# intuitive-robots/mdt_policy

Measured on AMD Instinct MI355X. Metric: action-chunks/sec (10-step denoise, horizon=10), higher is better.
Workload: dtype f32

## Files before the change

include/mdt_hip_ops.h:

```cpp
#ifndef MDT_HIP_OPS_H
#define MDT_HIP_OPS_H

#include <stdint.h>
#include "mdt_hip.h"

#ifdef __cplusplus
extern "C" {
#endif

enum { MDT_ACT_NONE = 0, MDT_ACT_GELU = 1, MDT_ACT_MISH = 2, MDT_ACT_SILU = 3,
       MDT_ACT_SWIGLU = 4  };
enum { MDT_HEAD_DENOISED = 0, MDT_HEAD_DDIM = 1, MDT_HEAD_RAW = 2,
       MDT_HEAD_PLAN = 3  };

int64_t mdt_op_packed_numel(int64_t N, int64_t K);

mdt_status mdt_op_pack_weight(const float *w, int64_t n_rows, int64_t K, float *packed, int64_t n_off,
                              int64_t N_total, void *stream);
mdt_status mdt_op_pack_weight_glu(const float *w, int64_t H2, int64_t K, float *packed, void *stream);

typedef struct {
    const float *A;
    int64_t lda;
    const float *Wp;
    const float *bias;
    float *out;
    int64_t ldo;
    int32_t M, N, K;
    int32_t ln;
    const float *ln_w, *ln_b;
    const float *mod;
    int64_t mod_stride;
    int32_t shift_off, scale_off;
    int32_t rows_per_sample;
    int32_t act;
    int32_t residual;
    int32_t gate_off;
    int32_t gin, gout, goff;
    const float *rowvec;
    int32_t batch;
    int64_t bs_a, bs_w, bs_out;
    const float *aux;
    int32_t aux_mode;
    int32_t a_parts;
    int64_t a_part_stride;
    float *a_merged;
    const void *Wp_split;
} mdt_gemm_args;

mdt_status mdt_op_gemm(const mdt_gemm_args *args, void *stream);

mdt_status mdt_op_mlp(const mdt_gemm_args *fc, const mdt_gemm_args *proj, float *parts, int64_t part_stride,
                      int32_t *n_parts, void *stream);
mdt_status mdt_op_pack_weight_split(const float *w, int64_t n_rows, int64_t K, void *image, void *stream);
mdt_status mdt_op_pack_weight_split_rows(const float *w, int64_t n_rows, int64_t K, void *image, int64_t n_off, void *stream);
mdt_status mdt_op_mlp_split(const mdt_gemm_args *fc, const mdt_gemm_args *proj, const void *fc_split, const void *proj_split,
                            float *parts, int64_t part_stride, int32_t *n_parts, void *stream);
void mdt_op_set_mlp_split(int32_t on);
void mdt_op_set_mlp_fuse_min(int32_t rows);
void mdt_op_set_side_jobs(int32_t on);
int64_t mdt_op_side_jobs_paired(void);
void mdt_op_trace_mlp(int32_t enable);
int32_t mdt_op_trace_mlp_read(float *us, int32_t cap);
int32_t mdt_op_trace_mlp_read_empty(float *us, int32_t cap);
mdt_status mdt_op_clock_stamp(uint64_t *out16, void *stream);
void mdt_op_set_ws_split(int32_t on);

void mdt_op_set_mlp_skew(int32_t v);

void mdt_op_set_gemm_geometry(int32_t geometry);

typedef struct {
    const float *q; int64_t ldq;
    const float *k; const float *v;
    int64_t ldkv;
    float *out; int64_t ldo;
    int32_t B, H, hd, Tq, Tk;
    int32_t causal;
    int32_t rope;
} mdt_attn_args;

mdt_status mdt_op_attention(const mdt_attn_args *args, void *stream);

mdt_status mdt_op_attn_proj(const mdt_gemm_args *proj, const float *qkv, int64_t ldq, int32_t hd, int32_t T, int32_t causal,
                            void *stream);
void mdt_op_set_attn_wide_min(int32_t rows);

mdt_status mdt_op_layernorm(const float *in, const float *w, const float *b, float *out, int64_t M, int32_t D,
                            void *stream);

typedef struct {
    const float *y;
    const float *ln_w;
    const float *ln_b;
    const float *Wp, *bp;
    const float *x;
    const float *sigma;
    int64_t sigma_stride;
    float *out;
    int32_t M, D, A, rows_per_sample;
    int32_t mode;
    const float *step;
    float sigma_data;
    float *y_next;
    const float *Wa, *ba;
    int32_t no_ln;
    int32_t y_parts;
    int64_t y_part_stride;
} mdt_head_args;

mdt_status mdt_op_head(const mdt_head_args *args, void *stream);

typedef struct {
    const float *kv; int64_t ldkv;
    const float *WqT_p;
    const float *bq;
    const float *Wo_p;
    float *U, *Wf;
    float *c;
    int32_t B, H, hd, D, Te;
} mdt_xfold_args;
mdt_status mdt_op_xattn_fold(const mdt_xfold_args *args, void *stream);

typedef struct {
    float *y;
    const float *ln_w, *ln_b;
    const float *U, *Wf, *c;
    const float *bo;
    int32_t B, H, D, Te, Ta;
    float *y_out;
} mdt_xapply_args;
mdt_status mdt_op_xattn_apply(const mdt_xapply_args *args, void *stream);

mdt_status mdt_op_xattn_gemm(const mdt_xapply_args *x, const mdt_gemm_args *g, void *stream);

mdt_status mdt_op_attn_xattn(const mdt_gemm_args *proj, const float *qkv, int64_t ldq, const mdt_xapply_args *x, int32_t hd,
                             int32_t T, void *stream);

mdt_status mdt_op_action_embed(const float *x, const float *sigma, int64_t sigma_stride, float sigma_data,
                               const float *WaT, const float *ba, float *y, int64_t M, int32_t A, int32_t D,
                               int32_t rows_per_sample, void *stream);
// ... 6 lines not shown
```

mdt_policy_amd/_lib.py:

```python
from __future__ import annotations

import ctypes as C
import os
import threading

from . import build as _build

c_float_p = C.POINTER(C.c_float)


class MDTHipError(RuntimeError):
    def __init__(self, status: int, message: str):
        super().__init__(f"libmdt_hip status {status}: {message}")
        self.status = status


class MDTConfig(C.Structure):
    _fields_ = [(n, C.c_int32) for n in (
        "arch", "embed_dim", "n_heads", "n_enc_layers", "n_dec_layers", "action_dim", "obs_dim", "goal_dim",
        "n_obs_token", "goal_seq_len", "action_seq_len", "use_mlp_goal", "use_modality_encoder", "use_abs_pos_emb",
        "use_rot_embed", "use_ada_conditioning", "use_noise_encoder", "linear_output", "bias")] + [
        ("sigma_data", C.c_float), ("no_goal_conditioning", C.c_int32), ("proprio_dim", C.c_int32),
        ("use_proprio", C.c_int32)]

# ... 146 lines not shown
class MapPoolConfig(C.Structure):
    _fields_ = [(n, C.c_int32) for n in ("n_latents", "embed_dim", "output_dim", "n_heads", "mlp_hidden")]


class InfoNCEArgs(C.Structure):
    _fields_ = [("image_features", C.c_void_p), ("lang_features", C.c_void_p), ("logit_scale", C.c_void_p),
                ("batch", C.c_int32), ("dim", C.c_int32), ("mode", C.c_int32), ("loss", C.c_void_p),
                ("d_image", C.c_void_p), ("d_lang", C.c_void_p), ("d_logit_scale", C.c_void_p), ("scratch", C.c_void_p)]


INFONCE_MODE = {"symmetric": 0, "img_to_text": 1, "text_to_img": 2}
ARCH = {"mdtv": 0, "mdt": 1}
MODALITY = {"vis": 0, "lang": 1}
ACT = {"none": 0, "gelu": 1, "mish": 2, "silu": 3, "swiglu": 4}
HEAD = {"denoised": 0, "ddim": 1, "raw": 2}
RAW_OUTPUT, RAW_INPUT, SIGMA_SCALAR = 1, 2, 4

_VP, _I32, _I64, _F = C.c_void_p, C.c_int32, C.c_int64, C.c_float
SYMBOLS = [
    ("mdt_last_error", C.c_char_p, []),
    ("mdt_version", C.c_char_p, []),
    ("mdt_set_allocator", _I32, [_VP, _VP, _VP]),
    ("mdt_allocator_detach", _I32, []),
    ("mdt_create", _I32, [C.POINTER(MDTConfig), C.POINTER(_VP)]),
    ("mdt_destroy", _I32, [_VP]),
    ("mdt_param_count", _I64, [_VP]),
    ("mdt_param_name", C.c_char_p, [_VP, _I64]),
    ("mdt_param_numel", _I64, [_VP, _I64]),
    ("mdt_load_param", _I32, [_VP, C.c_char_p, _VP, _I64, _VP]),
    ("mdt_load_params", _I32, [_VP, _I32, C.POINTER(C.c_char_p), C.POINTER(C.c_void_p), C.POINTER(_I64), _VP]),
    ("mdt_reserve", _I32, [_VP, _I64]),
    ("mdt_ws_generation", _I64, [_VP]),
    ("mdt_encode", _I32, [_VP, _VP, _VP, _VP, _I32, _I32, _VP, _I64, _VP, _VP]),
    ("mdt_denoise_cached", _I32, [_VP, _VP, _VP, _I64, _I32, _VP, _VP]),
    ("mdt_forward", _I32, [_VP, _VP, _VP, _VP, _I32, _VP, _VP, _I64, _VP, _VP, _VP]),
    ("mdt_sample_ddim", _I32, [_VP, _VP, _VP, _VP, _I32, _VP, C.POINTER(C.c_float), _I32, _I64, _VP, _VP, _VP]),
    ("mdt_sample_ddim_dev", _I32, [_VP, _VP, _VP, _VP, _I32, _VP, _VP, _I32, _I64, _VP, _VP, _VP]),
    ("mdt_sample", _I32, [_VP, _VP, _VP, _VP, _I32, _VP, _I32, C.POINTER(SamplerParams), C.POINTER(C.c_float), _I32, _VP, _I32,
                          _I64, _VP, _VP, _VP]),
    ("mdt_sample_dev", _I32, [_VP, _VP, _VP, _VP, _I32, _VP, _I32, C.POINTER(SamplerParams), _VP, _I32, _VP, _I32, _I64, _VP,
                              _VP, _VP]),
    ("mdt_sampler_plan", _I32, [_I32, C.POINTER(SamplerParams), C.POINTER(C.c_float), _I32, C.POINTER(SamplerPlan)]),
    ("mdt_sample_dpm_adaptive", _I32, [_VP, _VP, _VP, _VP, _I32, _VP, C.c_float, C.c_float, C.POINTER(DpmAdaptiveParams), _I64,
                                       _VP, _VP, C.POINTER(DpmAdaptiveInfo), _VP]),
    ("mdt_sample_ddim_guided", _I32, [_VP, _VP, _VP, _VP, _I32, _VP, C.POINTER(C.c_float), _I32, _I64, _VP, _VP, _F, _VP]),
    ("mdt_sample_ddim_dev_guided", _I32, [_VP, _VP, _VP, _VP, _I32, _VP, _VP, _I32, _I64, _VP, _VP, _F, _VP]),
    ("mdt_sample_guided", _I32, [_VP, _VP, _VP, _VP, _I32, _VP, _I32, C.POINTER(SamplerParams), C.POINTER(C.c_float), _I32, _VP,
                                 _I32, _I64, _VP, _VP, _F, _VP]),
    ("mdt_sample_dev_guided", _I32, [_VP, _VP, _VP, _VP, _I32, _VP, _I32, C.POINTER(SamplerParams), _VP, _I32, _VP, _I32, _I64,
                                     _VP, _VP, _F, _VP]),
    ("mdt_brownian_noise", _I32, [_VP, _I32, C.c_double, C.c_double, C.c_double, _VP, _I32, _I64, _I64, _VP, _VP]),
    ("mdt_brownian_noise_host", _I32, [_VP, _I32, C.c_double, C.c_double, C.c_double, _VP, _I32, _I64, _I64, _VP]),
    ("mdt_sample_sde_tree", _I32, [_VP, _VP, _VP, _VP, _I32, _VP, C.POINTER(SamplerParams), C.POINTER(C.c_float), _I32,
                                   C.POINTER(BrownianSource), _I64, _VP, _VP, _VP]),
    ("mdt_sample_sde_tree_dev", _I32, [_VP, _VP, _VP, _VP, _I32, _VP, C.POINTER(SamplerParams), _VP, _I32, C.POINTER(BrownianSource),
                                       _I64, _VP, _VP, _VP]),
    ("mdt_sample_sde_tree_guided", _I32, [_VP, _VP, _VP, _VP, _I32, _VP, C.POINTER(SamplerParams), C.POINTER(C.c_float), _I32,
                                          C.POINTER(BrownianSource), _I64, _VP, _VP, _F, _VP]),
    ("mdt_sample_sde_tree_dev_guided", _I32, [_VP, _VP, _VP, _VP, _I32, _VP, C.POINTER(SamplerParams), _VP, _I32,
                                              C.POINTER(BrownianSource), _I64, _VP, _VP, _F, _VP]),
    ("mdt_sample_dpm_adaptive_guided", _I32, [_VP, _VP, _VP, _VP, _I32, _VP, C.c_float, C.c_float, C.POINTER(DpmAdaptiveParams),
                                              _I64, _VP, _VP, _F, C.POINTER(DpmAdaptiveInfo), _VP]),
    ("mdt_dpm_control_init", _I32, [C.POINTER(DpmControl)] + [C.c_double] * 6),
    ("mdt_dpm_control_update", _I32, [C.POINTER(DpmControl), C.c_float, C.POINTER(C.c_int32)]),
    ("mdt_dpm_adaptive_plan", _I32, [_I32, C.c_float, C.c_float, C.POINTER(SamplerPlan)]),
    ("mdt_op_trace_mlp", None, [_I32]),
    ("mdt_op_trace_mlp_read", _I32, [_VP, _I32]),
    ("mdt_op_trace_mlp_read_empty", _I32, [_VP, _I32]),
    ("mdt_op_clock_stamp", _I32, [_VP, _VP]),
    ("mdt_op_set_ws_split", None, [_I32]),
    ("mdt_op_set_tn_split", None, [_I32]),
    ("mdt_loss_fwd", _I32, [_VP, _VP, _VP, _VP, _I32, _VP, _VP, _VP, _I64, _VP, _VP, _VP, _VP]),
    ("mdt_flops_per_chunk", C.c_double, [_VP, _I32]),
    ("mdt_fnv1_32", C.c_uint32, [C.c_char_p, C.c_uint64, C.c_uint32]),
    ("mdt_op_packed_numel", _I64, [_I64, _I64]),
    ("mdt_op_pack_weight", _I32, [_VP, _I64, _I64, _VP, _I64, _I64, _VP]),
    ("mdt_op_pack_weight_glu", _I32, [_VP, _I64, _I64, _VP, _VP]),
    ("mdt_op_gemm", _I32, [C.POINTER(GemmArgs), _VP]),
    ("mdt_op_mlp", _I32, [C.POINTER(GemmArgs), C.POINTER(GemmArgs), _VP, _I64, C.POINTER(_I32), _VP]),
    ("mdt_op_pack_weight_split", _I32, [_VP, _I64, _I64, _VP, _VP]),
    ("mdt_op_pack_weight_split_rows", _I32, [_VP, _I64, _I64, _VP, _I64, _VP]),
    ("mdt_op_mlp_split", _I32, [C.POINTER(GemmArgs), C.POINTER(GemmArgs), _VP, _VP, _VP, _I64, C.POINTER(_I32), _VP]),
    ("mdt_op_set_mlp_split", None, [_I32]),
    ("mdt_op_set_gemm_geometry", None, [_I32]),
    ("mdt_op_set_mlp_fuse_min", None, [_I32]),
    ("mdt_op_set_side_jobs", None, [_I32]),
    ("mdt_op_side_jobs_paired", _I64, []),
    ("mdt_op_set_mlp_skew", None, [_I32]),
    ("mdt_op_set_attn_wide_min", None, [_I32]),
    ("mdt_op_attention", _I32, [C.POINTER(AttnArgs), _VP]),
    ("mdt_op_attn_proj", _I32, [C.POINTER(GemmArgs), _VP, _I64, _I32, _I32, _I32, _VP]),
    ("mdt_op_xattn_fold", _I32, [C.POINTER(XFoldArgs), _VP]),
    ("mdt_op_xattn_apply", _I32, [C.POINTER(XApplyArgs), _VP]),
    ("mdt_op_attn_xattn", _I32, [C.POINTER(GemmArgs), _VP, _I64, C.POINTER(XApplyArgs), _I32, _I32, _VP]),
    ("mdt_op_xattn_gemm", _I32, [C.POINTER(XApplyArgs), C.POINTER(GemmArgs), _VP]),
    ("mdt_op_layernorm", _I32, [_VP, _VP, _VP, _VP, _I64, _I32, _VP]),
    ("mdt_op_head", _I32, [C.POINTER(HeadArgs), _VP]),
    ("mdt_op_action_embed", _I32, [_VP, _VP, _I64, _F, _VP, _VP, _VP, _I64, _I32, _I32, _I32, _VP]),
    ("mdt_train_prepare", _I32, [_VP]),
    ("mdt_grad_numel", _I64, [_VP]),
    ("mdt_grad_offset", _I64, [_VP, _I64]),
    ("mdt_train_loss_fwd", _I32, [_VP, _VP, _VP, _VP, _I32, _VP, _VP, _VP, _I64, C.POINTER(Dropout), _VP, _VP, _VP,
                                  C.POINTER(_I32), _VP]),
    ("mdt_train_loss_bwd", _I32, [_VP, _I32, _VP, _VP, _VP, _VP, _VP, _VP, _VP]),
    ("mdt_train_loss_bwd_stages", _I32, [_VP]),
    ("mdt_train_loss_bwd_stage", _I32, [_VP, _I32, _I32, _VP, _VP, _VP, _VP, _VP, _VP, _VP]),
    ("mdt_train_param_stage", _I32, [_VP, _I64]),
    ("mdt_train_encode_fwd", _I32, [_VP, _VP, _VP, _VP, _I32, _I32, _VP, _I64, C.POINTER(Dropout), _VP, C.POINTER(_I32),
                                    _VP]),
    ("mdt_train_encode_bwd", _I32, [_VP, _I32, _VP, _VP, _VP, _VP, _VP, _VP]),
    ("mdt_tape_release", _I32, [_VP, _I32]),
    ("mdt_denoise_vjp", _I32, [_VP, _VP, _VP, _VP, _I32, _VP, _VP, _VP, _I64, _VP, _VP, _VP]),
    ("mdt_train_denoise_fwd", _I32, [_VP, _VP, _VP, _VP, _I64, C.POINTER(Dropout), _VP, C.POINTER(_I32), _VP]),
    ("mdt_train_denoise_bwd", _I32, [_VP, _I32, _VP, _VP, _VP, _VP, _VP, _VP]),
    ("mdt_op_pack_weight_t", _I32, [_VP, _I64, _I64, _I64, _VP, _I64, _I64, _VP]),
    ("mdt_op_pack_many", _I32, [_I32, C.POINTER(C.c_void_p), C.POINTER(_I32), C.POINTER(_I32), C.POINTER(C.c_void_p),
                                C.POINTER(C.c_void_p), _VP]),
    ("mdt_op_ln_fwd_train", _I32, [C.POINTER(LnTrainArgs), _VP]),
    ("mdt_op_ln_bwd", _I32, [C.POINTER(LnBwdArgs), _VP]),
    ("mdt_op_attn_bwd", _I32, [C.POINTER(AttnBwdArgs), _VP]),
    ("mdt_op_act_fwd", _I32, [_VP, _VP, _I64, _I32, _VP]),
    ("mdt_op_act_bwd", _I32, [_VP, _VP, _VP, _I64, _I32, _VP]),
    ("mdt_op_attn_fwd_train", _I32, [C.POINTER(AttnTrainArgs), _VP]),
    ("mdt_op_merge_fwd", _I32, [C.POINTER(MergeArgs), _VP]),
    ("mdt_op_merge_bwd", _I32, [C.POINTER(MergeArgs), _VP]),
    ("mdt_op_merge_ln_fwd", _I32, [C.POINTER(MergeArgs), C.POINTER(LnTrainArgs), _VP]),
    ("mdt_op_ln_bwd_merge", _I32, [C.POINTER(LnBwdArgs), C.POINTER(MergeArgs), _VP]),
    ("mdt_op_colsum", _I32, [_VP, _I64, _I64, _I64, _VP, _I32, _VP]),
    ("mdt_op_linear_bwd", _I32, [C.POINTER(LinearBwdArgs), _VP]),
    ("mdt_op_linear_bwd_scratch", _I64, [_I64, _I64, _I64]),
    ("mdt_op_linear_bwd_scratch_exact", _I64, [_I64, _I64, _I64]),
    ("mdt_op_multi_adamw", _I32, [C.POINTER(OptTensor), _I32, _F, _F, _F, _F, _F, _I64, _VP]),
    ("mdt_op_multi_ema", _I32, [C.POINTER(OptTensor), _I32, _F, _VP]),
    ("mdt_op_multi_sumsq_scratch", _I64, [C.POINTER(OptTensor), _I32]),
    ("mdt_op_multi_sumsq", _I32, [C.POINTER(OptTensor), _I32, _I32, _VP, _VP, _I64, _VP]),
    ("mdt_op_multi_adamw_dev", _I32, [C.POINTER(OptTensor), _I32, _F, _F, _F, _F, _F, _VP, _VP, _VP, _VP, _F, _VP, _VP]),
    ("mdt_resampler_create", _I32, [C.POINTER(ResamplerConfig), C.POINTER(_VP)]),
    ("mdt_resampler_destroy", _I32, [_VP]),
    ("mdt_resampler_param_count", _I64, [_VP]),
    ("mdt_resampler_param_name", C.c_char_p, [_VP, _I64]),
    ("mdt_resampler_param_numel", _I64, [_VP, _I64]),
    ("mdt_resampler_load_param", _I32, [_VP, C.c_char_p, _VP, _I64, _VP]),
    ("mdt_resampler_forward", _I32, [_VP, _VP, _VP, _I64, _I32, _I32, _VP, _VP]),
    ("mdt_resampler_train_prepare", _I32, [_VP]),
    ("mdt_resampler_grad_numel", _I64, [_VP]),
    ("mdt_resampler_grad_offset", _I64, [_VP, _I64]),
    ("mdt_resampler_forward_train", _I32, [_VP, _VP, _VP, _I64, _I32, _I32, _VP, C.POINTER(_I32), _VP]),
    ("mdt_resampler_backward", _I32, [_VP, _I32, _VP, _VP, _VP, _VP]),
    ("mdt_resampler_tape_release", _I32, [_VP, _I32]),
    ("mdt_resampler_flops", C.c_double, [_VP, _I32, _I32]),
    ("mdt_map_pool_create", _I32, [C.POINTER(MapPoolConfig), C.POINTER(_VP)]),
    ("mdt_map_pool_destroy", _I32, [_VP]),
    ("mdt_map_pool_param_count", _I64, [_VP]),
    ("mdt_map_pool_param_name", C.c_char_p, [_VP, _I64]),
    ("mdt_map_pool_param_numel", _I64, [_VP, _I64]),
    ("mdt_map_pool_load_param", _I32, [_VP, C.c_char_p, _VP, _I64, _VP]),
    ("mdt_map_pool_forward", _I32, [_VP, _VP, _I64, _I32, _VP, _VP]),
    ("mdt_map_pool_train_prepare", _I32, [_VP]),
    ("mdt_map_pool_grad_numel", _I64, [_VP]),
    ("mdt_map_pool_grad_offset", _I64, [_VP, _I64]),
    ("mdt_map_pool_forward_train", _I32, [_VP, _VP, _I64, _I32, _VP, C.POINTER(_I32), _VP]),
    ("mdt_map_pool_backward", _I32, [_VP, _I32, _VP, _VP, _VP, _VP]),
    ("mdt_map_pool_tape_release", _I32, [_VP, _I32]),
    ("mdt_op_rms_fwd", _I32, [_VP, _VP, _VP, _I64, _I32, _F, _VP]),
    ("mdt_op_rms_bwd_scratch", _I64, [_I64, _I32]),
    ("mdt_op_rms_bwd", _I32, [_VP, _VP, _VP, _VP, _I32, _VP, _I32, _I64, _I32, _F, _VP, _VP]),
# ... 131 lines not shown
```

mdt_policy_amd/csrc/mdt_kernels.hip:

```cpp
#include <hip/hip_runtime.h>

#include <atomic>
#include <stdint.h>
#include <stdlib.h>

#include <mutex>
#include <vector>

#include "mdt_internal.h"

#include "mdt_device.h"

#define MDT_TILES_TIMING_OWNER
#include "mdt_tiles.h"
#include "mdt_sampler_plan.h"
#include "mdt_tall.h"
#include "mdt_ws.h"
#include "mdt_mlp_split.h"

__global__ void k_pack_weight(const float* __restrict__ w, int n_rows, int K, float* __restrict__ packed,
                              int n_off, int K16) {
    const int64_t idx = (int64_t)blockIdx.x * blockDim.x + threadIdx.x;
    if (idx >= (int64_t)n_rows * K) return;
    const int n = (int)(idx / K), k = (int)(idx % K);
// ... 829 lines not shown
    if (a.M >= 8192 && (a.aux_mode == 0 || a.K == 384) && g_mdt_gemm_force <= 0 && mdt_gemm_ws_supported(a)) return launch_gemm_ws(a, s);
    if (a.M >= 8192 && a.N % 64 == 0 && (a.N > 384 || a.K > 384) && a.batch <= 1 && mdt_gemm_tall_supported(a)) geo = 23;
    if (a.batch > 1) geo = 5;
    if (g_mdt_gemm_force > 0) geo = g_mdt_gemm_force;
    if (geo == 30) {
        if (mdt_gemm_ws_supported(a)) return launch_gemm_ws(a, s);
        geo = 0;
    }
    if (geo >= 10 && (geo != 23 || !mdt_gemm_tall_supported(a))) geo = 0;
    switch (geo) {
        case 23: return launch_gemm_tall<2, 2, 2, 3, 1>(a, s);
        case 1: return launch_gemm_pro<2, 1, 4>(a, mdt_gemm_kchunk(a.K, a.ln, 384), s);
        case 2:
            if (!a.ln && a.K > 512) {
                const int kc = mdt_gemm_kchunk(a.K, 0, 384);
                return a.residual ? launch_gemm_pipe_r<2, 1, 8, 4, true>(a, kc, s)
                                  : launch_gemm_pipe_r<2, 1, 8, 4, false>(a, kc, s);
            }
            return launch_gemm_pro<2, 1, 8>(a, mdt_gemm_kchunk(a.K, a.ln, 768), s);
        case 3: return launch_gemm_pro<2, 3, 8>(a, mdt_gemm_kchunk(a.K, a.ln, 768), s);
        case 4: return launch_gemm_pro<2, 4, 8>(a, mdt_gemm_kchunk(a.K, a.ln, 768), s);
        case 6: {
            if (!a.ln && a.K > 512 && !a.aux_mode && (int64_t)((a.M + 15) / 16) * ((a.N + 63) / 64) <= 256) {
                const int kc = mdt_gemm_kchunk(a.K, 0, 384);
                return a.residual ? launch_gemm_pipe_r<1, 1, 4, 2, true>(a, kc, s) : launch_gemm_pipe_r<1, 1, 4, 2, false>(a, kc, s);
            }
            return launch_gemm_pro<1, 1, 4>(a, mdt_gemm_kchunk(a.K, a.ln, 384), s);
        }
        case 7: return launch_gemm_pro<4, 2, 4>(a, mdt_gemm_kchunk(a.K, a.ln, 384), s);
        case 8: return launch_gemm_pro<2, 4, 4>(a, mdt_gemm_kchunk(a.K, a.ln, 384), s);
        case 9: return launch_gemm_pro<2, 3, 4>(a, mdt_gemm_kchunk(a.K, a.ln, 384), s);
        default: return launch_gemm_pro<2, 2, 4>(a, mdt_gemm_kchunk(a.K, a.ln, 384), s);
    }
}

extern "C" void mdt_op_set_gemm_geometry(int32_t geo) { g_mdt_gemm_force = geo; }

bool mdt_mlp_supported(const mdt_gemm_args& f, const mdt_gemm_args& p) {
    const int D = f.K;
    return D >= 128 && D <= 512 && D % 128 == 0 && f.N == 4 * D && p.N == D && p.K == 4 * D && f.ln && f.batch <= 1 &&
           f.gin == 1 && f.gout == 1 && f.goff == 0 && f.rowvec == nullptr && !f.aux_mode && f.a_parts <= 1 && f.M >= 1 &&
           f.rows_per_sample >= 1 && p.rows_per_sample >= 1;
}
int mdt_mlp_slices(int D) { return 4 * D / 512; }

static int g_mlp_skew = -1;
static int mlp_skew() { return g_mlp_skew < 0 ? 18 | 256 : g_mlp_skew; }
extern "C" void mdt_op_set_mlp_skew(int32_t v) { g_mlp_skew = v < 0 ? -1 : (v & 0x1ff); }

template <int NTW2, int PRO>
static hipError_t launch_mlp_t(const mdt_gemm_args& f, const mdt_gemm_args& p, float* parts, int64_t part_stride, hipStream_t s) {
    const int S = mdt_mlp_slices(f.K), gm = (f.M + 31) / 32;
    const size_t lds = (size_t)32 * (f.K + 4 + 516) * sizeof(float) + 16 * sizeof(int);
    const int skew = mlp_skew();
    static size_t lds_attr_dev[MAX_DEVICES] = {0};
    size_t& lds_attr = lds_attr_dev[current_device()];
    if (lds > lds_attr) {
        hipError_t e = hipFuncSetAttribute((const void*)k_mlp<NTW2, PRO>, hipFuncAttributeMaxDynamicSharedMemorySize, (int)lds);
        if (e != hipSuccess) return e;
        lds_attr = lds;
    }
    hipLaunchKernelGGL((k_mlp<NTW2, PRO>), dim3(gm * S), dim3(512), lds, s, f, p, parts, part_stride, S, g_zeros, skew);
    return hipGetLastError();
}
template <int NTW2>
static hipError_t launch_mlp_pro(const mdt_gemm_args& f, const mdt_gemm_args& p, float* parts, int64_t part_stride, hipStream_t s) {
    if (f.mod != nullptr && f.shift_off >= 0)
        return f.mod_stride == 0 ? launch_mlp_t<NTW2, PRO_LN_MOD_BCAST>(f, p, parts, part_stride, s)
                                 : launch_mlp_t<NTW2, PRO_LN_MOD_ROWS>(f, p, parts, part_stride, s);
    return launch_mlp_t<NTW2, PRO_LN>(f, p, parts, part_stride, s);
}
hipError_t mdt_launch_mlp(const mdt_gemm_args& f, const mdt_gemm_args& p, float* parts, int64_t part_stride, hipStream_t s) {
    if (!mdt_mlp_supported(f, p)) return hipErrorInvalidValue;
    hipError_t ze = ensure_zeros();
    if (ze != hipSuccess) return ze;
    switch (f.K / 128) {
        case 1: return launch_mlp_pro<1>(f, p, parts, part_stride, s);
        case 2: return launch_mlp_pro<2>(f, p, parts, part_stride, s);
        case 3: return launch_mlp_pro<3>(f, p, parts, part_stride, s);
        default: return launch_mlp_pro<4>(f, p, parts, part_stride, s);
    }
}

template <int ND, int NTW, int PRO, int XP>
__global__ __launch_bounds__(512) void k_gemm_ln_split(mdt_gemm_args a, int grid_n, const float* __restrict__ zeros) {
    extern __shared__ __attribute__((aligned(16))) char lds_c[];
    const int logical = xcd_remap(blockIdx.x, gridDim.x);
    const int by = logical / grid_n, bx = logical - by * grid_n;
    gemm_ln_split_tile<ND, NTW, PRO, XP>(a, by, bx, lds_c, zeros, threadIdx.x);
}
template <int ND, int NTW, int PRO, int XP>
static hipError_t launch_gemm_ln_split_t(const mdt_gemm_args& a, hipStream_t s) {
    const int gn = a.N / (8 * NTW * 16), gm = (a.M + 31) / 32;
    const int lds = 3 * 32 * (2 * 128 * ND + 32);
    static bool attr_dev[MAX_DEVICES] = {false};
    bool& done = attr_dev[current_device()];
    if (!done) {
        hipError_t e = hipFuncSetAttribute((const void*)k_gemm_ln_split<ND, NTW, PRO, XP>, hipFuncAttributeMaxDynamicSharedMemorySize, lds);
        if (e != hipSuccess) return e;
        done = true;
    }
    hipLaunchKernelGGL((k_gemm_ln_split<ND, NTW, PRO, XP>), dim3(gn * gm), dim3(512), lds, s, a, gn, g_zeros);
    return hipGetLastError();
}
template <int ND, int NTW, int PRO>
static hipError_t launch_gemm_ln_split_x(const mdt_gemm_args& a, hipStream_t s) {
    switch (a.a_parts) {
        case 2: return launch_gemm_ln_split_t<ND, NTW, PRO, 2>(a, s);
        case 3: return launch_gemm_ln_split_t<ND, NTW, PRO, 3>(a, s);
        case 4: return launch_gemm_ln_split_t<ND, NTW, PRO, 4>(a, s);
        default: return launch_gemm_ln_split_t<ND, NTW, PRO, 1>(a, s);
    }
}
template <int ND, int NTW>
static hipError_t launch_gemm_ln_split_pro(const mdt_gemm_args& a, hipStream_t s) {
    if (a.mod != nullptr && a.shift_off >= 0)
        return a.mod_stride == 0 ? launch_gemm_ln_split_x<ND, NTW, PRO_LN_MOD_BCAST>(a, s) : launch_gemm_ln_split_x<ND, NTW, PRO_LN_MOD_ROWS>(a, s);
    return launch_gemm_ln_split_x<ND, NTW, PRO_LN>(a, s);
}
static bool gemm_ln_split_applies(const mdt_gemm_args& a) {
    return a.Wp_split != nullptr && mdt_mlp_split_enabled() && a.ln && (a.K == 384 || a.K == 512) && a.N % 384 == 0 &&
           a.M >= mdt_split_min_rows() && a.batch <= 1 && !a.residual && a.gin == 1 && a.gout == 1 && a.goff == 0 && a.rowvec == nullptr && !a.aux_mode &&
           a.a_parts <= 4 && (a.lda & 3) == 0 && (a.ldo & 3) == 0 && g_mdt_gemm_force == 0;
}
static hipError_t launch_gemm_ln_split(const mdt_gemm_args& a, hipStream_t s) {
    return a.K == 512 ? launch_gemm_ln_split_pro<4, 3>(a, s) : launch_gemm_ln_split_pro<3, 3>(a, s);
}

static int g_mlp_split = -1;
bool mdt_mlp_split_enabled() {
    if (g_mlp_split < 0) { const char* e = getenv("MDT_HIP_MLP_SPLIT"); g_mlp_split = e ? atoi(e) : 1; }
    return g_mlp_split != 0;
}
extern "C" void mdt_op_set_mlp_split(int32_t on) { g_mlp_split = on < 0 ? -1 : (on != 0); }
int mdt_split_min_rows() { return 768; }
bool mdt_mlp_split_supported(const mdt_gemm_args& f, const mdt_gemm_args& p) {
    return mdt_mlp_supported(f, p);
}
template <int NTW2, int PRO>
static hipError_t launch_mlp_split_t(const mdt_gemm_args& f, const mdt_gemm_args& p, const void* w1s, const void* w2s, float* parts,
                                     int64_t part_stride, hipStream_t s) {
    const int S = mdt_mlp_slices(f.K), gm = (f.M + 31) / 32;
    const int lds = mlp_split_lds_bytes(128 * NTW2);
    static bool attr_dev[MAX_DEVICES] = {false};
    bool& done = attr_dev[current_device()];
    if (!done) {
        hipError_t e = hipFuncSetAttribute((const void*)k_mlp_split<NTW2, PRO>, hipFuncAttributeMaxDynamicSharedMemorySize, lds);
        if (e != hipSuccess) return e;
        done = true;
    }
    const int per = (gm * S + 7) / 8;
    hipLaunchKernelGGL((k_mlp_split<NTW2, PRO>), dim3(8 * per), dim3(512), lds, s, f, p, (const char*)w1s, (const char*)w2s, parts,
                       part_stride, S, gm, g_zeros);
    return hipGetLastError();
}
template <int NTW2>
static hipError_t launch_mlp_split_pro(const mdt_gemm_args& f, const mdt_gemm_args& p, const void* w1s, const void* w2s, float* parts,
                                       int64_t part_stride, hipStream_t s) {
    if (f.mod != nullptr && f.shift_off >= 0)
        return f.mod_stride == 0 ? launch_mlp_split_t<NTW2, PRO_LN_MOD_BCAST>(f, p, w1s, w2s, parts, part_stride, s)
                                 : launch_mlp_split_t<NTW2, PRO_LN_MOD_ROWS>(f, p, w1s, w2s, parts, part_stride, s);
    return launch_mlp_split_t<NTW2, PRO_LN>(f, p, w1s, w2s, parts, part_stride, s);
}
hipError_t mdt_launch_mlp_split(const mdt_gemm_args& f, const mdt_gemm_args& p, const void* w1s, const void* w2s, float* parts,
                                int64_t part_stride, hipStream_t s) {
    if (!mdt_mlp_split_supported(f, p) || !w1s || !w2s) return hipErrorInvalidValue;
    hipError_t ze = ensure_zeros();
    if (ze != hipSuccess) return ze;
    switch (f.K / 128) {
        case 1: return launch_mlp_split_pro<1>(f, p, w1s, w2s, parts, part_stride, s);
        case 2: return launch_mlp_split_pro<2>(f, p, w1s, w2s, parts, part_stride, s);
        case 3: return launch_mlp_split_pro<3>(f, p, w1s, w2s, parts, part_stride, s);
        default: return launch_mlp_split_pro<4>(f, p, w1s, w2s, parts, part_stride, s);
    }
}

template <int NTW, int PRO, int XP>
static hipError_t launch_gemm_merge_t(const mdt_gemm_args& a, hipStream_t s) {
    const int NTC = 8 * NTW * 16;
    const int gn = (a.N + NTC - 1) / NTC, gm = (a.M + 31) / 32;
    const size_t lds = (size_t)32 * (a.K + 4) * sizeof(float);
    static size_t lds_attr_dev[MAX_DEVICES] = {0};
    size_t& lds_attr = lds_attr_dev[current_device()];
    if (lds > lds_attr) {
        hipError_t e = hipFuncSetAttribute((const void*)k_gemm_merge<NTW, PRO, XP>, hipFuncAttributeMaxDynamicSharedMemorySize, (int)lds);
        if (e != hipSuccess) return e;
        lds_attr = lds;
    }
    hipLaunchKernelGGL((k_gemm_merge<NTW, PRO, XP>), dim3(gn * gm), dim3(512), lds, s, a, a.K, gn, g_zeros);
    return hipGetLastError();
}
template <int NTW, int PRO>
static hipError_t launch_gemm_merge_x(const mdt_gemm_args& a, hipStream_t s) {
    switch (a.a_parts) {
        case 2: return launch_gemm_merge_t<NTW, PRO, 2>(a, s);
        case 3: return launch_gemm_merge_t<NTW, PRO, 3>(a, s);
        case 4: return launch_gemm_merge_t<NTW, PRO, 4>(a, s);
        default: return hipErrorInvalidValue;
    }
}
template <int NTW>
static hipError_t launch_gemm_merge_pro(const mdt_gemm_args& a, hipStream_t s) {
    if (a.mod != nullptr && a.shift_off >= 0)
        return a.mod_stride == 0 ? launch_gemm_merge_x<NTW, PRO_LN_MOD_BCAST>(a, s) : launch_gemm_merge_x<NTW, PRO_LN_MOD_ROWS>(a, s);
    return launch_gemm_merge_x<NTW, PRO_LN>(a, s);
}
static hipError_t launch_gemm_merge(const mdt_gemm_args& a, hipStream_t s) {
    if (!a.ln || a.K > 512 || a.residual || a.batch > 1 || a.aux_mode || a.a_parts > 4 || (a.N & 15)) return hipErrorInvalidValue;
    return (a.N % 384 == 0) ? launch_gemm_merge_pro<3>(a, s) : launch_gemm_merge_pro<4>(a, s);
// ... 851 lines not shown
```

mdt_policy_amd/csrc/mdt_mlp_split.h:

```cpp
#pragma once
#include <hip/hip_runtime.h>
#include <stdint.h>

#include "mdt_device.h"
#include "mdt_internal.h"
#include "mdt_tiles.h"
#include "mdt_ws.h"

template <int NT, int R>
struct SplitRing {
    mdt_bf16x8 w[R][NT][3];
    __amdgpu_buffer_rsrc_t rs;
    unsigned voff[NT];
    __device__ __forceinline__ void open(const void* image, int64_t first_byte, int64_t tile_stride, int lane) {
        rs = __builtin_amdgcn_make_buffer_rsrc((void*)image, 0, 0xffffffffu, 0x00020000);
#pragma unroll
        for (int j = 0; j < NT; ++j) voff[j] = (unsigned)(first_byte + j * tile_stride) + 16u * (unsigned)lane;
    }
    __device__ __forceinline__ void request(int slot, int kk) {
#pragma unroll
        for (int j = 0; j < NT; ++j)
#pragma unroll
            for (int p = 0; p < 3; ++p)
                w[slot][j][p] = __builtin_bit_cast(mdt_bf16x8, __builtin_amdgcn_raw_buffer_load_b128(rs, voff[j], (kk * 3 + p) * 1024, 0));
// ... 83 lines not shown
    SplitRing<NTW1, R> ring1;
    ring1.open(w1s, (int64_t)nt1 * K32a * 3072, (int64_t)K32a * 3072, lane);
#pragma unroll
    for (int u = 0; u < R - 1; ++u) ring1.request(u, u);
    f32x4 b1[NTW1];
    {
        const float* bp = f.bias != nullptr ? f.bias : zeros;
#pragma unroll
        for (int j = 0; j < NTW1; ++j) b1[j] = ldg4(bp + (nt1 + j) * 16 + nq);
    }
    gemm_stage_tile<MTILES, NWAVES, PRO, false, 1, 2, true>(f, (float*)xs, ROWB1, m0, 0, D, zeros, tid, lane, wave);
    __syncthreads();
    f32x4 acc1[MTILES][NTW1];
#pragma unroll
    for (int i = 0; i < MTILES; ++i)
#pragma unroll
        for (int j = 0; j < NTW1; ++j) acc1[i][j] = zero4;
    split_phase<NTW1, K32a, R>(ring1, xs, ROWB1, PART1, lane, acc1);

    const int K32p = p.K >> 5;
    SplitRing<NTW2, R> ring2;
    ring2.open(w2s, ((int64_t)(wave * NTW2) * K32p + (int64_t)s * K32b) * 3072, (int64_t)K32p * 3072, lane);
#pragma unroll
    for (int u = 0; u < R - 1; ++u) ring2.request(u, u);
    constexpr bool EARLY = NTW2 <= 3;
    f32x4 acc2[MTILES][NTW2], b2[NTW2], gate_v[MTILES][NTW2], res_v[MTILES][NTW2];
    int ncol[NTW2];
#pragma unroll
    for (int j = 0; j < NTW2; ++j) ncol[j] = (wave * NTW2 + j) * 16 + nq;
    const bool gated = p.mod != nullptr && p.gate_off >= 0;
    auto load_gate_res = [&]() __attribute__((always_inline)) {
#pragma unroll
        for (int i = 0; i < MTILES; ++i) {
            const int64_t m = min(m0 + i * 16 + (lane & 15), f.M - 1);
            const float* gp = gated ? p.mod + p.gate_off + (p.mod_stride == 0 ? 0 : (m / p.rows_per_sample) * p.mod_stride)
                                    : zeros;
            const float* rp = s == 0 ? f.A + m * f.lda : zeros;
#pragma unroll
            for (int j = 0; j < NTW2; ++j) {
                gate_v[i][j] = ldg4(gp + ncol[j]);
                res_v[i][j] = ldg4(rp + ncol[j]);
            }
        }
    };
    {
        const float* bp = (s == 0 && p.bias != nullptr) ? p.bias : zeros;
#pragma unroll
        for (int j = 0; j < NTW2; ++j) b2[j] = ldg4(bp + ncol[j]);
#pragma unroll
        for (int i = 0; i < MTILES; ++i)
#pragma unroll
            for (int j = 0; j < NTW2; ++j) acc2[i][j] = zero4;
        if constexpr (EARLY) load_gate_res();
    }
    __syncthreads();
#pragma unroll
    for (int i = 0; i < MTILES; ++i)
#pragma unroll
        for (int j = 0; j < NTW1; ++j) {
            mdt_bf16x4 p1, p2, p3;
            split3_bf16(apply_act(acc1[i][j] + b1[j], f.act), p1, p2, p3);
            char* q = hs + split_slot(i * 16 + (lane & 15), (wave * NTW1 + j) * 16 + nq, ROWB2);
            *(mdt_bf16x4*)q = p1;
            *(mdt_bf16x4*)(q + PART2) = p2;
            *(mdt_bf16x4*)(q + 2 * PART2) = p3;
        }
    __syncthreads();
    split_phase<NTW2, K32b, R>(ring2, hs, ROWB2, PART2, lane, acc2);

    if constexpr (!EARLY) load_gate_res();
    float* out = parts + (int64_t)s * part_stride;
#pragma unroll
    for (int i = 0; i < MTILES; ++i) {
        const int m = m0 + i * 16 + (lane & 15);
#pragma unroll
        for (int j = 0; j < NTW2; ++j) {
            f32x4 v = acc2[i][j] + b2[j];
            v = res_v[i][j] + (gated ? gate_v[i][j] * v : v);
            if (m < f.M) st4(out + (int64_t)m * p.ldo + ncol[j], v);
        }
    }
}

template <int ND, int NTW, int PRO, int XP>
__device__ __forceinline__ void gemm_ln_split_tile(const mdt_gemm_args& a, int by, int bx, char* lds, const float* __restrict__ zeros, int tid) {
    constexpr int MTILES = 2, NWAVES = 8, MT = 32, R = 2;
    constexpr int D = 128 * ND, K32 = D / 32, ROWB = 2 * D + 32, PART = MT * ROWB;
    static_assert(ND >= 1 && ND <= 4, "D <= 512");
    const f32x4 zero4 = (f32x4){0.f, 0.f, 0.f, 0.f};
    const int lane = tid & 63, wave = tid >> 6;
    const int m0 = by * MT, nq = 4 * (lane >> 4);
    char* xs = lds;
    const int nt0 = (bx * NWAVES + wave) * NTW;
    SplitRing<NTW, R> ring;
    ring.open(a.Wp_split, (int64_t)nt0 * K32 * 3072, (int64_t)K32 * 3072, lane);
#pragma unroll
    for (int u = 0; u < R - 1; ++u) ring.request(u, u);
    f32x4 bias_v[NTW];
    {
        const float* bp = a.bias != nullptr ? a.bias : zeros;
#pragma unroll
        for (int j = 0; j < NTW; ++j) bias_v[j] = ldg4(bp + (nt0 + j) * 16 + nq);
    }
    gemm_stage_tile<MTILES, NWAVES, PRO, false, XP, (NTW <= 3 && XP <= 3) ? 1 : 2, true>(a, (float*)xs, ROWB, m0, 0, D, zeros, tid, lane, wave,
                                                                                         bx == 0 ? a.a_merged : nullptr);
    __syncthreads();
    f32x4 acc[MTILES][NTW];
#pragma unroll
    for (int i = 0; i < MTILES; ++i)
#pragma unroll
        for (int j = 0; j < NTW; ++j) acc[i][j] = zero4;
    split_phase<NTW, K32, R>(ring, xs, ROWB, PART, lane, acc);
#pragma unroll
    for (int i = 0; i < MTILES; ++i) {
        const int m = m0 + i * 16 + (lane & 15);
#pragma unroll
        for (int j = 0; j < NTW; ++j)
            if (m < a.M) st4(a.out + (int64_t)m * a.ldo + (nt0 + j) * 16 + nq, apply_act(acc[i][j] + bias_v[j], a.act));
    }
}
```

Baseline: 74750.

## Use narrower 192-column panels for small LN-split GEMM grids

Adds a panel-width template parameter to the LayerNorm-fused split GEMM, so that only PW of the eight staging waves perform the multiply and each block covers fewer output columns. When the grid would be small (single A part and at most 256 blocks at 192 columns), it uses 6 multiplying waves with 2 tiles each, doubling the block count to fill more compute units. Idle waves still help stage the normalized tile and then exit, and LDS is padded to limit occupancy per CU. A setter is added to force the panel choice. The trade-off is redundant LN staging per block and more blocks re-reading the activation tile.

```diff
diff --git a/include/mdt_hip_ops.h b/include/mdt_hip_ops.h
--- a/include/mdt_hip_ops.h
+++ b/include/mdt_hip_ops.h
@@ -57,6 +57,7 @@
 mdt_status mdt_op_mlp_split(const mdt_gemm_args *fc, const mdt_gemm_args *proj, const void *fc_split, const void *proj_split,
                             float *parts, int64_t part_stride, int32_t *n_parts, void *stream);
 void mdt_op_set_mlp_split(int32_t on);
+void mdt_op_set_split_panel(int32_t cols);
 void mdt_op_set_mlp_fuse_min(int32_t rows);
 void mdt_op_set_side_jobs(int32_t on);
 int64_t mdt_op_side_jobs_paired(void);
diff --git a/mdt_policy_amd/_lib.py b/mdt_policy_amd/_lib.py
--- a/mdt_policy_amd/_lib.py
+++ b/mdt_policy_amd/_lib.py
@@ -252,6 +252,7 @@
     ("mdt_op_pack_weight_split_rows", _I32, [_VP, _I64, _I64, _VP, _I64, _VP]),
     ("mdt_op_mlp_split", _I32, [C.POINTER(GemmArgs), C.POINTER(GemmArgs), _VP, _VP, _VP, _I64, C.POINTER(_I32), _VP]),
     ("mdt_op_set_mlp_split", None, [_I32]),
+    ("mdt_op_set_split_panel", None, [_I32]),
     ("mdt_op_set_gemm_geometry", None, [_I32]),
     ("mdt_op_set_mlp_fuse_min", None, [_I32]),
     ("mdt_op_set_side_jobs", None, [_I32]),
diff --git a/mdt_policy_amd/csrc/mdt_kernels.hip b/mdt_policy_amd/csrc/mdt_kernels.hip
--- a/mdt_policy_amd/csrc/mdt_kernels.hip
+++ b/mdt_policy_amd/csrc/mdt_kernels.hip
@@ -935,49 +935,58 @@
     }
 }
 
-template <int ND, int NTW, int PRO, int XP>
+template <int ND, int NTW, int PRO, int XP, int PW>
 __global__ __launch_bounds__(512) void k_gemm_ln_split(mdt_gemm_args a, int grid_n, const float* __restrict__ zeros) {
     extern __shared__ __attribute__((aligned(16))) char lds_c[];
     const int logical = xcd_remap(blockIdx.x, gridDim.x);
     const int by = logical / grid_n, bx = logical - by * grid_n;
-    gemm_ln_split_tile<ND, NTW, PRO, XP>(a, by, bx, lds_c, zeros, threadIdx.x);
-}
-template <int ND, int NTW, int PRO, int XP>
+    gemm_ln_split_tile<ND, NTW, PRO, XP, PW>(a, by, bx, lds_c, zeros, threadIdx.x);
+}
+template <int ND, int NTW, int PRO, int XP, int PW>
 static hipError_t launch_gemm_ln_split_t(const mdt_gemm_args& a, hipStream_t s) {
-    const int gn = a.N / (8 * NTW * 16), gm = (a.M + 31) / 32;
-    const int lds = 3 * 32 * (2 * 128 * ND + 32);
+    const int gn = a.N / (PW * NTW * 16), gm = (a.M + 31) / 32;
+    const int tile = 3 * 32 * (2 * 128 * ND + 32), lds = PW < 8 && tile < 84 * 1024 ? 84 * 1024 : tile;
     static bool attr_dev[MAX_DEVICES] = {false};
     bool& done = attr_dev[current_device()];
     if (!done) {
-        hipError_t e = hipFuncSetAttribute((const void*)k_gemm_ln_split<ND, NTW, PRO, XP>, hipFuncAttributeMaxDynamicSharedMemorySize, lds);
+        hipError_t e = hipFuncSetAttribute((const void*)k_gemm_ln_split<ND, NTW, PRO, XP, PW>, hipFuncAttributeMaxDynamicSharedMemorySize, lds);
         if (e != hipSuccess) return e;
         done = true;
     }
-    hipLaunchKernelGGL((k_gemm_ln_split<ND, NTW, PRO, XP>), dim3(gn * gm), dim3(512), lds, s, a, gn, g_zeros);
-    return hipGetLastError();
-}
-template <int ND, int NTW, int PRO>
+    hipLaunchKernelGGL((k_gemm_ln_split<ND, NTW, PRO, XP, PW>), dim3(gn * gm), dim3(512), lds, s, a, gn, g_zeros);
+    return hipGetLastError();
+}
+template <int ND, int NTW, int PRO, int PW>
 static hipError_t launch_gemm_ln_split_x(const mdt_gemm_args& a, hipStream_t s) {
     switch (a.a_parts) {
-        case 2: return launch_gemm_ln_split_t<ND, NTW, PRO, 2>(a, s);
-        case 3: return launch_gemm_ln_split_t<ND, NTW, PRO, 3>(a, s);
-        case 4: return launch_gemm_ln_split_t<ND, NTW, PRO, 4>(a, s);
-        default: return launch_gemm_ln_split_t<ND, NTW, PRO, 1>(a, s);
-    }
-}
-template <int ND, int NTW>
+        case 2: return launch_gemm_ln_split_t<ND, NTW, PRO, 2, PW>(a, s);
+        case 3: return launch_gemm_ln_split_t<ND, NTW, PRO, 3, PW>(a, s);
+        case 4: return launch_gemm_ln_split_t<ND, NTW, PRO, 4, PW>(a, s);
+        default: return launch_gemm_ln_split_t<ND, NTW, PRO, 1, PW>(a, s);
+    }
+}
+template <int ND, int NTW, int PW>
 static hipError_t launch_gemm_ln_split_pro(const mdt_gemm_args& a, hipStream_t s) {
     if (a.mod != nullptr && a.shift_off >= 0)
-        return a.mod_stride == 0 ? launch_gemm_ln_split_x<ND, NTW, PRO_LN_MOD_BCAST>(a, s) : launch_gemm_ln_split_x<ND, NTW, PRO_LN_MOD_ROWS>(a, s);
-    return launch_gemm_ln_split_x<ND, NTW, PRO_LN>(a, s);
+        return a.mod_stride == 0 ? launch_gemm_ln_split_x<ND, NTW, PRO_LN_MOD_BCAST, PW>(a, s) : launch_gemm_ln_split_x<ND, NTW, PRO_LN_MOD_ROWS, PW>(a, s);
+    return launch_gemm_ln_split_x<ND, NTW, PRO_LN, PW>(a, s);
 }
 static bool gemm_ln_split_applies(const mdt_gemm_args& a) {
     return a.Wp_split != nullptr && mdt_mlp_split_enabled() && a.ln && (a.K == 384 || a.K == 512) && a.N % 384 == 0 &&
            a.M >= mdt_split_min_rows() && a.batch <= 1 && !a.residual && a.gin == 1 && a.gout == 1 && a.goff == 0 && a.rowvec == nullptr && !a.aux_mode &&
            a.a_parts <= 4 && (a.lda & 3) == 0 && (a.ldo & 3) == 0 && g_mdt_gemm_force == 0;
 }
+static std::atomic<int> g_split_panel{0};
+extern "C" void mdt_op_set_split_panel(int32_t cols) { g_split_panel.store(cols == 384 || cols == 192 ? cols : 0); }
+static int gemm_ln_split_panel(const mdt_gemm_args& a) {
+    const int forced = g_split_panel.load(std::memory_order_relaxed);
+    if (forced) return forced;
+    const int64_t gm = (a.M + 31) / 32;
+    return a.a_parts <= 1 && gm * (a.N / 192) <= 256 ? 192 : 384;
+}
 static hipError_t launch_gemm_ln_split(const mdt_gemm_args& a, hipStream_t s) {
-    return a.K == 512 ? launch_gemm_ln_split_pro<4, 3>(a, s) : launch_gemm_ln_split_pro<3, 3>(a, s);
+    if (gemm_ln_split_panel(a) == 192) return a.K == 512 ? launch_gemm_ln_split_pro<4, 2, 6>(a, s) : launch_gemm_ln_split_pro<3, 2, 6>(a, s);
+    return a.K == 512 ? launch_gemm_ln_split_pro<4, 3, 8>(a, s) : launch_gemm_ln_split_pro<3, 3, 8>(a, s);
 }
 
 static int g_mlp_split = -1;
diff --git a/mdt_policy_amd/csrc/mdt_mlp_split.h b/mdt_policy_amd/csrc/mdt_mlp_split.h
--- a/mdt_policy_amd/csrc/mdt_mlp_split.h
+++ b/mdt_policy_amd/csrc/mdt_mlp_split.h
@@ -189,7 +189,7 @@
     }
 }
 
-template <int ND, int NTW, int PRO, int XP>
+template <int ND, int NTW, int PRO, int XP, int PW = 8>
 __device__ __forceinline__ void gemm_ln_split_tile(const mdt_gemm_args& a, int by, int bx, char* lds, const float* __restrict__ zeros, int tid) {
     constexpr int MTILES = 2, NWAVES = 8, MT = 32, R = 2;
     constexpr int D = 128 * ND, K32 = D / 32, ROWB = 2 * D + 32, PART = MT * ROWB;
@@ -198,13 +198,15 @@
     const int lane = tid & 63, wave = tid >> 6;
     const int m0 = by * MT, nq = 4 * (lane >> 4);
     char* xs = lds;
-    const int nt0 = (bx * NWAVES + wave) * NTW;
+    static_assert(PW >= 1 && PW <= NWAVES, "the multiplying waves are among the staging waves");
+    const int nt0 = (bx * PW + wave) * NTW;
+    const bool mul = PW == NWAVES || wave < PW;
     SplitRing<NTW, R> ring;
-    ring.open(a.Wp_split, (int64_t)nt0 * K32 * 3072, (int64_t)K32 * 3072, lane);
-#pragma unroll
-    for (int u = 0; u < R - 1; ++u) ring.request(u, u);
     f32x4 bias_v[NTW];
-    {
+    if (mul) {
+        ring.open(a.Wp_split, (int64_t)nt0 * K32 * 3072, (int64_t)K32 * 3072, lane);
+#pragma unroll
+        for (int u = 0; u < R - 1; ++u) ring.request(u, u);
         const float* bp = a.bias != nullptr ? a.bias : zeros;
 #pragma unroll
         for (int j = 0; j < NTW; ++j) bias_v[j] = ldg4(bp + (nt0 + j) * 16 + nq);
@@ -212,6 +214,7 @@
     gemm_stage_tile<MTILES, NWAVES, PRO, false, XP, (NTW <= 3 && XP <= 3) ? 1 : 2, true>(a, (float*)xs, ROWB, m0, 0, D, zeros, tid, lane, wave,
                                                                                          bx == 0 ? a.a_merged : nullptr);
     __syncthreads();
+    if (!mul) return;
     f32x4 acc[MTILES][NTW];
 #pragma unroll
     for (int i = 0; i < MTILES; ++i)
```

New measurement: 75600 (median of 4 runs). 1.1% higher.
